# srv902/FOCUS

Hardware: AMD Instinct MI355X
Metric: clips/sec (fwd+bwd+opt step) ORViT-MF 16x224 (higher is better)
Workload: dtype bf16; 1 GPU; ORViT-Motionformer 16x224, 4 objects, batch=8 per GPU (BASELINE configs[1]); global_batch=8, frames=16, crop=224, objects=4, parallelism=dp1, optimizer=adamw+clipnorm

## Files before the change

focus_amd/csrc/gemm_tn_group.hip:

```cpp
#include "focus_common.h"
#include "gemm_internal.h"
#include <algorithm>

namespace {

typedef __attribute__((ext_vector_type(8))) __bf16 bf16x8;
typedef __attribute__((ext_vector_type(4))) short s16x4;
typedef __attribute__((ext_vector_type(4))) float f32x4;
typedef __attribute__((address_space(1))) const void gvoid_t;
typedef __attribute__((address_space(3))) void lvoid_t;
typedef __attribute__((address_space(3))) s16x4 lds_s16x4;

constexpr int BKM = 64;
constexpr int SUB = BKM * 256;
constexpr int NSTAGE = 3, NLOAD = 4;
constexpr int BI = 256, BJ = 128;

union Frag { bf16x8 v; s16x4 t[2]; uint32_t u[4]; };

__device__ __forceinline__ int swz(int row) { return ((row & 3) | ((row >> 1) & 4)) << 1; }
__device__ __forceinline__ int toff(int row, int col) {
    return row * 256 + ((((col >> 3)) ^ swz(row)) << 4) + (col & 4) * 2;
}
__device__ __forceinline__ bf16x8 col_frag16(const char* tile, int r0, int c0, int lane) {
    const int i = lane & 15;
    const int row = r0 + (i >> 2), col = c0 + 4 * (i & 3);
    Frag f;
    f.t[0] = __builtin_amdgcn_ds_read_tr16_b64_v4i16((lds_s16x4*)(tile + toff(row, col)));
    f.t[1] = __builtin_amdgcn_ds_read_tr16_b64_v4i16((lds_s16x4*)(tile + toff(row + 4, col)));
    return f.v;
}

struct Prob {
    const bf16_t* P;
    const bf16_t* Q;
    float* C;
    float* db;
    int64_t ldp, ldq;
    int32_t I, J, Mred, tiles_i, tiles_j, pad_;
};
constexpr int MAXP = 8;
struct GroupArgs { Prob p[MAXP]; int32_t nprob, nunits; };
struct UnitRec { int16_t prob, ti, tj, pad_; };

__global__ __launch_bounds__(64 * (BI * BJ / 4096 + NLOAD)) void gemm_tn_group_kernel(const GroupArgs ga, const UnitRec* __restrict__ units) {
    constexpr int NCONS = BI * BJ / 4096;
    constexpr int WJ = BJ / 64;
    constexpr int NSP = BI / 128, NSQ = BJ / 128, NSUBT = NSP + NSQ;
    constexpr int STAGE = NSUBT * SUB;
    constexpr int PIECES = NSUBT * 16 / NLOAD;
    extern __shared__ __attribute__((aligned(16))) char smem[];

    const int tid = threadIdx.x, lane = tid & 63;
    const int w = __builtin_amdgcn_readfirstlane(tid >> 6);
    const int nunits = ga.nunits;
    const int G = gridDim.x, xcd = blockIdx.x & 7, jwg = blockIdx.x >> 3;
    const int gx = (G >> 3) + (xcd < (G & 7) ? 1 : 0);
    const int q8 = nunits >> 3, r8 = nunits & 7;
    const int band0 = xcd < r8 ? xcd * (q8 + 1) : r8 * (q8 + 1) + (xcd - r8) * q8;
    const int band_n = q8 + (xcd < r8 ? 1 : 0);
    const int my_units = jwg < band_n ? (band_n - jwg + gx - 1) / gx : 0;
    if (my_units == 0) return;

    struct Unit { const bf16_t* P; const bf16_t* Q; float* C; float* db; int64_t ldp, ldq; int I, J, Mred, i0, j0, nk, valid_last, tj; };
    auto unit_of = [&](int i) __attribute__((always_inline)) {
        const UnitRec ur = units[band0 + jwg + i * gx];
        const int pi = __builtin_amdgcn_readfirstlane((int)ur.prob);
        Unit t;
        Prob p = ga.p[0];
#pragma unroll
        for (int k = 1; k < MAXP; ++k)
            if (pi == k) p = ga.p[k];
        t.P = p.P; t.Q = p.Q; t.C = p.C; t.db = p.db; t.ldp = p.ldp; t.ldq = p.ldq; t.I = p.I; t.J = p.J; t.Mred = p.Mred;
        t.i0 = __builtin_amdgcn_readfirstlane((int)ur.ti) * BI;
        t.tj = __builtin_amdgcn_readfirstlane((int)ur.tj);
        t.j0 = t.tj * BJ;
        t.nk = (p.Mred + BKM - 1) / BKM;
        t.valid_last = p.Mred - (t.nk - 1) * BKM;
        return t;
    };

    if (w >= NCONS) {
        const int L = w - NCONS;
        const int cpos = lane & 15, rin = lane >> 4;
        Unit cur = unit_of(0);
        int iu = 0, ikt = 0;
        auto issue = [&](int st) __attribute__((always_inline)) {
            char* sp = smem + st * STAGE;
            const int mb = ikt * BKM;
#pragma unroll
            for (int g = 0; g < PIECES; ++g) {
                const int sub = g >> 2, pi = g * NLOAD + L, row = (pi & 15) * 4 + rin;
                const int m = min(mb + row, cur.Mred - 1);
                const int ch = cpos ^ swz(row);
                const bf16_t* src;
                if (sub < NSP) src = cur.P + (int64_t)m * cur.ldp + min(cur.i0 + sub * 128 + ch * 8, cur.I - 8);
                else src = cur.Q + (int64_t)m * cur.ldq + min(cur.j0 + (sub - NSP) * 128 + ch * 8, cur.J - 8);
                __builtin_amdgcn_global_load_lds((gvoid_t*)src, (lvoid_t*)(sp + pi * 1024), 16, 0, 0);
            }
            if (++ikt == cur.nk) { ikt = 0; if (++iu < my_units) cur = unit_of(iu); }
        };
        int total = 0;
        for (int i = 0; i < my_units; ++i) total += unit_of(i).nk;
        issue(0);
        if (total > 1) {
            issue(1);
            asm volatile("s_waitcnt vmcnt(%0)" ::"n"(PIECES) : "memory");
        } else {
            asm volatile("s_waitcnt vmcnt(0)" ::: "memory");
        }
        __builtin_amdgcn_s_barrier();
        int st2 = 2;
        for (int t = 0; t < total; ++t) {
            if (t + 2 < total) {
                issue(st2);
                st2 = st2 == 2 ? 0 : st2 + 1;
                asm volatile("s_waitcnt vmcnt(%0)" ::"n"(PIECES) : "memory");
            } else {
                asm volatile("s_waitcnt vmcnt(0)" ::: "memory");
            }
            __builtin_amdgcn_s_barrier();
        }
        return;
    }

    const int wi = w / WJ, wj = w % WJ;
    const int fr = lane & 15, fq = lane >> 4;
    const int poff = (wi >> 1) * SUB, pcol = (wi & 1) * 64;
    const int qoff = (NSP + (wj >> 1)) * SUB, qcol = (wj & 1) * 64;
    f32x4 acc[4][4];
    constexpr int NA = 4 / WJ;
    f32x4 accb[NA];
    Frag ones;
    ones.u[0] = ones.u[1] = ones.u[2] = ones.u[3] = 0x3F803F80u;
    auto compute = [&](const char* stage, auto masked, int valid, bool cs) __attribute__((always_inline)) {
        const char* sp = stage + poff;
        const char* sq = stage + qoff;
#pragma unroll
        for (int ks = 0; ks < 2; ++ks) {
            bf16x8 fp[4], fqv[4];
#pragma unroll
            for (int a = 0; a < 4; ++a) fp[a] = col_frag16(sp, ks * 32 + 8 * fq, pcol + a * 16, lane);
#pragma unroll
            for (int b = 0; b < 4; ++b) fqv[b] = col_frag16(sq, ks * 32 + 8 * fq, qcol + b * 16, lane);
            if constexpr (decltype(masked)::value) {
                const int left = valid - (ks * 32 + 8 * fq);
#pragma unroll
                for (int a = 0; a < 4; ++a) {
                    Frag f; f.v = fp[a];
#pragma unroll
                    for (int e2 = 0; e2 < 4; ++e2) {
                        const uint32_t keep = (2 * e2 < left ? 0x0000ffffu : 0u) | (2 * e2 + 1 < left ? 0xffff0000u : 0u);
                        f.u[e2] &= keep;
                    }
                    fp[a] = f.v;
                }
            }
#pragma unroll
            for (int a = 0; a < 4; ++a)
#pragma unroll
                for (int b = 0; b < 4; ++b)
                    acc[a][b] = __builtin_amdgcn_mfma_f32_16x16x32_bf16(fqv[b], fp[a], acc[a][b], 0, 0, 0);
            if (cs) {
#pragma unroll
                for (int n = 0; n < NA; ++n) {
                    bf16x8 sel = fp[n];
#pragma unroll
                    for (int j = 1; j < WJ; ++j)
                        if (wj == j) sel = fp[j * NA + n];
                    accb[n] = __builtin_amdgcn_mfma_f32_16x16x32_bf16(ones.v, sel, accb[n], 0, 0, 0);
                }
            }
        }
    };

    __builtin_amdgcn_s_barrier();
    int st = 0;
    for (int cu = 0; cu < my_units; ++cu) {
        const Unit cur = unit_of(cu);
#pragma unroll
        for (int a = 0; a < 4; ++a)
#pragma unroll
            for (int b = 0; b < 4; ++b) acc[a][b] = (f32x4){0.f, 0.f, 0.f, 0.f};
        const bool want_b = cur.db != nullptr && cur.tj == 0;
#pragma unroll
        for (int n = 0; n < NA; ++n) accb[n] = (f32x4){0.f, 0.f, 0.f, 0.f};
        for (int kt = 0; kt + 1 < cur.nk; ++kt) {
            compute(smem + st * STAGE, std::false_type{}, BKM, want_b);
            st = st == 2 ? 0 : st + 1;
            __builtin_amdgcn_s_barrier();
        }
        compute(smem + st * STAGE, std::true_type{}, cur.valid_last, want_b);
        st = st == 2 ? 0 : st + 1;
        __builtin_amdgcn_s_barrier();
        if (want_b && fq == 0) {
#pragma unroll
            for (int n = 0; n < NA; ++n) {
                const int gi = cur.i0 + wi * 64 + (wj * NA + n) * 16 + fr;
                if (gi < cur.I) cur.db[gi] = accb[n][0];
            }
        }
#pragma unroll
        for (int a = 0; a < 4; ++a) {
            const int gi = cur.i0 + wi * 64 + a * 16 + fr;
            if (gi >= cur.I) continue;
#pragma unroll
            for (int b = 0; b < 4; ++b) {
                const int gj = cur.j0 + wj * 64 + b * 16 + fq * 4;
                if (gj < cur.J)
                    *reinterpret_cast<float4*>(cur.C + (int64_t)gi * cur.J + gj) =
                        make_float4(acc[a][b][0], acc[a][b][1], acc[a][b][2], acc[a][b][3]);
            }
        }
    }
}

}

extern "C" int focus_linear_wgrad_group_units(const focus_wgrad_item* items, int n_items) {
    if (!items || n_items <= 0) return 0;
    int64_t t = 0;
    for (int p = 0; p < n_items; ++p) t += (int64_t)((items[p].N + BI - 1) / BI) * ((items[p].K + BJ - 1) / BJ);
    return t > 0x7fffffff ? -1 : (int)t;
}

extern "C" int focus_linear_wgrad_group_plan(const focus_wgrad_item* items, int n_items, void* host_units, size_t bytes) {
    if (!items || !host_units) return FOCUS_ERR_NULL;
    if (n_items <= 0 || n_items > MAXP) return FOCUS_ERR_SHAPE;
    const int total = focus_linear_wgrad_group_units(items, n_items);
    if (total <= 0 || bytes < (size_t)total * sizeof(UnitRec)) return FOCUS_ERR_WORKSPACE;
    UnitRec* u = static_cast<UnitRec*>(host_units);
    constexpr int BA = 4, BB = 8;
    int n = 0;
    for (int p = 0; p < n_items; ++p) {
        const int ti_n = (items[p].N + BI - 1) / BI, tj_n = (items[p].K + BJ - 1) / BJ;
        for (int bi = 0; bi < ti_n; bi += BA)
            for (int bj = 0; bj < tj_n; bj += BB)
                for (int ti = bi; ti < std::min(bi + BA, ti_n); ++ti)
                    for (int tj = bj; tj < std::min(bj + BB, tj_n); ++tj)
                        u[n++] = UnitRec{(int16_t)p, (int16_t)ti, (int16_t)tj, 0};
    }
    return n == total ? FOCUS_OK : FOCUS_ERR_SHAPE;
}

extern "C" int focus_linear_wgrad_group(const focus_wgrad_item* items, int n_items, const void* dev_units, void* stream) {
    if (!items || !dev_units) return FOCUS_ERR_NULL;
    if (n_items <= 0) return FOCUS_OK;
    if (n_items > MAXP) return FOCUS_ERR_SHAPE;
    GroupArgs ga = {};
    int units = 0;
    for (int p = 0; p < n_items; ++p) {
        const focus_wgrad_item& it = items[p];
        if (!it.dy || !it.x || !it.dw) return FOCUS_ERR_NULL;
        if (it.M <= 0 || it.N < 8 || it.K < 8 || (it.N & 7) || (it.K & 7) || (it.ld_dy & 7) || (it.ld_x & 7)) return FOCUS_ERR_SHAPE;
        if (!focus_aligned(it.dy, 16) || !focus_aligned(it.x, 16) || !focus_aligned(it.dw, 16)) return FOCUS_ERR_ALIGN;
        Prob& q = ga.p[p];
        q.P = static_cast<const bf16_t*>(it.dy); q.Q = static_cast<const bf16_t*>(it.x);
        q.C = it.dw; q.db = it.db; q.ldp = it.ld_dy; q.ldq = it.ld_x;
        q.I = it.N; q.J = it.K; q.Mred = it.M;
        q.tiles_i = (it.N + BI - 1) / BI; q.tiles_j = (it.K + BJ - 1) / BJ; q.pad_ = 0;
        if (q.tiles_i > 32767 || q.tiles_j > 32767) return FOCUS_ERR_SHAPE;
        units += q.tiles_i * q.tiles_j;
    }
    ga.nprob = n_items;
    ga.nunits = units;
    hipStream_t s = static_cast<hipStream_t>(stream);
    const size_t lds = (size_t)NSTAGE * (BI / 128 + BJ / 128) * SUB;
    auto k = gemm_tn_group_kernel;
    static bool once = (hipFuncSetAttribute((const void*)k, hipFuncAttributeMaxDynamicSharedMemorySize, lds) == hipSuccess);
    (void)once;
    hipLaunchKernelGGL(k, dim3(std::min(units, 256)), dim3(64 * (BI * BJ / 4096 + NLOAD)), lds, s, ga,
                       static_cast<const UnitRec*>(dev_units));
    FOCUS_CHECK_LAUNCH();
    return FOCUS_OK;
}
```

Baseline: 299.1 clips/s.

## Precompute loader offsets, index problem table via kernarg, stage epilogue through LDS

The loader waves now compute per-row byte offsets once per unit and advance them by a fixed stride each k-step, clamping rows only on the last tile. This removes the per-load index arithmetic and the upfront pass that summed all units' k-tiles. The problem table is read directly from the kernel-argument segment using scalar reads instead of a select chain, and the bias path is made a compile-time branch. The output epilogue goes through a per-wave swizzled LDS slab so stores become coalesced nontemporal row writes, at the cost of extra LDS and waits.

Result: faster. 306.5 clips/s (median of 6 runs) (+2.5%).

```diff
diff --git a/focus_amd/csrc/gemm_tn_group.hip b/focus_amd/csrc/gemm_tn_group.hip
--- a/focus_amd/csrc/gemm_tn_group.hip
+++ b/focus_amd/csrc/gemm_tn_group.hip
@@ -1,6 +1,7 @@
 #include "focus_common.h"
 #include "gemm_internal.h"
 #include <algorithm>
+#include <cstddef>
 
 namespace {
 
@@ -15,6 +16,7 @@
 constexpr int SUB = BKM * 256;
 constexpr int NSTAGE = 3, NLOAD = 4;
 constexpr int BI = 256, BJ = 128;
+constexpr int SLAB = 2048;
 
 union Frag { bf16x8 v; s16x4 t[2]; uint32_t u[4]; };
 
@@ -29,6 +31,11 @@
     f.t[0] = __builtin_amdgcn_ds_read_tr16_b64_v4i16((lds_s16x4*)(tile + toff(row, col)));
     f.t[1] = __builtin_amdgcn_ds_read_tr16_b64_v4i16((lds_s16x4*)(tile + toff(row + 4, col)));
     return f.v;
+}
+
+__device__ __forceinline__ uint64_t uni64(uint64_t v) {
+    return ((uint64_t)(uint32_t)__builtin_amdgcn_readfirstlane((int)(v >> 32)) << 32) |
+           (uint32_t)__builtin_amdgcn_readfirstlane((int)(uint32_t)v);
 }
 
 struct Prob {
@@ -64,62 +71,116 @@
 
     struct Unit { const bf16_t* P; const bf16_t* Q; float* C; float* db; int64_t ldp, ldq; int I, J, Mred, i0, j0, nk, valid_last, tj; };
     auto unit_of = [&](int i) __attribute__((always_inline)) {
-        const UnitRec ur = units[band0 + jwg + i * gx];
-        const int pi = __builtin_amdgcn_readfirstlane((int)ur.prob);
+        const uint2 raw = reinterpret_cast<const uint2*>(units)[band0 + jwg + i * gx];
+        const int pi = __builtin_amdgcn_readfirstlane((int)(raw.x & 0xffffu)) & (MAXP - 1);
         Unit t;
-        Prob p = ga.p[0];
-#pragma unroll
-        for (int k = 1; k < MAXP; ++k)
-            if (pi == k) p = ga.p[k];
-        t.P = p.P; t.Q = p.Q; t.C = p.C; t.db = p.db; t.ldp = p.ldp; t.ldq = p.ldq; t.I = p.I; t.J = p.J; t.Mred = p.Mred;
-        t.i0 = __builtin_amdgcn_readfirstlane((int)ur.ti) * BI;
-        t.tj = __builtin_amdgcn_readfirstlane((int)ur.tj);
+        static_assert(offsetof(GroupArgs, p) == 0, "the problem table must open the kernel-argument segment");
+        typedef __attribute__((address_space(4))) const Prob karg_prob_t;
+        const karg_prob_t& p = ((const karg_prob_t*)__builtin_amdgcn_kernarg_segment_ptr())[pi];
+        t.P = reinterpret_cast<const bf16_t*>(uni64(reinterpret_cast<uint64_t>(p.P)));
+        t.Q = reinterpret_cast<const bf16_t*>(uni64(reinterpret_cast<uint64_t>(p.Q)));
+        t.C = reinterpret_cast<float*>(uni64(reinterpret_cast<uint64_t>(p.C)));
+        t.db = reinterpret_cast<float*>(uni64(reinterpret_cast<uint64_t>(p.db)));
+        t.ldp = (int64_t)uni64((uint64_t)p.ldp); t.ldq = (int64_t)uni64((uint64_t)p.ldq);
+        t.I = __builtin_amdgcn_readfirstlane(p.I); t.J = __builtin_amdgcn_readfirstlane(p.J);
+        t.Mred = __builtin_amdgcn_readfirstlane(p.Mred);
+        t.i0 = __builtin_amdgcn_readfirstlane((int)(raw.x >> 16)) * BI;
+        t.tj = __builtin_amdgcn_readfirstlane((int)(raw.y & 0xffffu));
         t.j0 = t.tj * BJ;
-        t.nk = (p.Mred + BKM - 1) / BKM;
-        t.valid_last = p.Mred - (t.nk - 1) * BKM;
+        t.nk = (t.Mred + BKM - 1) / BKM;
+        t.valid_last = t.Mred - (t.nk - 1) * BKM;
         return t;
     };
 
     if (w >= NCONS) {
         const int L = w - NCONS;
         const int cpos = lane & 15, rin = lane >> 4;
-        Unit cur = unit_of(0);
+        constexpr int GP = NSP * 4, GQ = NSQ * 4;
+        uint32_t p_off[GP], q_off[GQ];
+        const char* p_cur = nullptr;
+        const char* q_cur = nullptr;
+        int64_t p_step = 0, q_step = 0;
+        uint32_t ldp2 = 0, ldq2 = 0;
+        int nk = 0, Mred = 0;
         int iu = 0, ikt = 0;
+        bool more = true;
+        auto rowk = [&](int k) __attribute__((always_inline)) { return (k * NLOAD + L) * 4 + rin; };
+        auto setup = [&](int i) __attribute__((always_inline)) {
+            const Unit t = unit_of(i);
+            p_cur = reinterpret_cast<const char*>(t.P);
+            q_cur = reinterpret_cast<const char*>(t.Q);
+            p_step = t.ldp * (2 * BKM);
+            q_step = t.ldq * (2 * BKM);
+            ldp2 = 2u * (uint32_t)t.ldp;
+            ldq2 = 2u * (uint32_t)t.ldq;
+            nk = t.nk;
+            Mred = t.Mred;
+#pragma unroll
+            for (int k = 0; k < 4; ++k) {
+                const int row = rowk(k), ch = cpos ^ swz(row);
+#pragma unroll
+                for (int s = 0; s < NSP; ++s)
+                    p_off[s * 4 + k] = (uint32_t)row * ldp2 + 2u * (uint32_t)min(t.i0 + s * 128 + ch * 8, t.I - 8);
+#pragma unroll
+                for (int s = 0; s < NSQ; ++s)
+                    q_off[s * 4 + k] = (uint32_t)row * ldq2 + 2u * (uint32_t)min(t.j0 + s * 128 + ch * 8, t.J - 8);
+            }
+        };
         auto issue = [&](int st) __attribute__((always_inline)) {
             char* sp = smem + st * STAGE;
-            const int mb = ikt * BKM;
-#pragma unroll
-            for (int g = 0; g < PIECES; ++g) {
-                const int sub = g >> 2, pi = g * NLOAD + L, row = (pi & 15) * 4 + rin;
-                const int m = min(mb + row, cur.Mred - 1);
-                const int ch = cpos ^ swz(row);
-                const bf16_t* src;
-                if (sub < NSP) src = cur.P + (int64_t)m * cur.ldp + min(cur.i0 + sub * 128 + ch * 8, cur.I - 8);
-                else src = cur.Q + (int64_t)m * cur.ldq + min(cur.j0 + (sub - NSP) * 128 + ch * 8, cur.J - 8);
-                __builtin_amdgcn_global_load_lds((gvoid_t*)src, (lvoid_t*)(sp + pi * 1024), 16, 0, 0);
-            }
-            if (++ikt == cur.nk) { ikt = 0; if (++iu < my_units) cur = unit_of(iu); }
+            if (ikt + 1 < nk) {
+#pragma unroll
+                for (int g = 0; g < GP; ++g)
+                    __builtin_amdgcn_global_load_lds((gvoid_t*)(p_cur + p_off[g]), (lvoid_t*)(sp + (g * NLOAD + L) * 1024), 16, 0, 0);
+#pragma unroll
+                for (int g = 0; g < GQ; ++g)
+                    __builtin_amdgcn_global_load_lds((gvoid_t*)(q_cur + q_off[g]), (lvoid_t*)(sp + ((GP + g) * NLOAD + L) * 1024), 16, 0, 0);
+                p_cur += p_step;
+                q_cur += q_step;
+                ++ikt;
+            } else {
+                const int last = Mred - 1 - ikt * BKM;
+                uint32_t pb[4], qb[4];
+#pragma unroll
+                for (int k = 0; k < 4; ++k) {
+                    const uint32_t over = (uint32_t)max(rowk(k) - last, 0);
+                    pb[k] = over * ldp2;
+                    qb[k] = over * ldq2;
+                }
+#pragma unroll
+                for (int g = 0; g < GP; ++g)
+                    __builtin_amdgcn_global_load_lds((gvoid_t*)(p_cur + (p_off[g] - pb[g & 3])), (lvoid_t*)(sp + (g * NLOAD + L) * 1024), 16, 0, 0);
+#pragma unroll
+                for (int g = 0; g < GQ; ++g)
+                    __builtin_amdgcn_global_load_lds((gvoid_t*)(q_cur + (q_off[g] - qb[g & 3])), (lvoid_t*)(sp + ((GP + g) * NLOAD + L) * 1024), 16, 0, 0);
+                ikt = 0;
+                if (++iu < my_units) setup(iu);
+                else more = false;
+            }
         };
-        int total = 0;
-        for (int i = 0; i < my_units; ++i) total += unit_of(i).nk;
+        setup(0);
         issue(0);
-        if (total > 1) {
+        int pending = 1;
+        if (more) {
             issue(1);
+            ++pending;
             asm volatile("s_waitcnt vmcnt(%0)" ::"n"(PIECES) : "memory");
         } else {
             asm volatile("s_waitcnt vmcnt(0)" ::: "memory");
         }
         __builtin_amdgcn_s_barrier();
         int st2 = 2;
-        for (int t = 0; t < total; ++t) {
-            if (t + 2 < total) {
+        while (pending > 0) {
+            if (more) {
                 issue(st2);
+                ++pending;
                 st2 = st2 == 2 ? 0 : st2 + 1;
                 asm volatile("s_waitcnt vmcnt(%0)" ::"n"(PIECES) : "memory");
             } else {
                 asm volatile("s_waitcnt vmcnt(0)" ::: "memory");
             }
             __builtin_amdgcn_s_barrier();
+            --pending;
         }
         return;
     }
@@ -133,7 +194,7 @@
     f32x4 accb[NA];
     Frag ones;
     ones.u[0] = ones.u[1] = ones.u[2] = ones.u[3] = 0x3F803F80u;
-    auto compute = [&](const char* stage, auto masked, int valid, bool cs) __attribute__((always_inline)) {
+    auto compute = [&](const char* stage, auto masked, int valid, auto cs) __attribute__((always_inline)) {
         const char* sp = stage + poff;
         const char* sq = stage + qoff;
 #pragma unroll
@@ -161,7 +222,7 @@
 #pragma unroll
                 for (int b = 0; b < 4; ++b)
                     acc[a][b] = __builtin_amdgcn_mfma_f32_16x16x32_bf16(fqv[b], fp[a], acc[a][b], 0, 0, 0);
-            if (cs) {
+            if constexpr (decltype(cs)::value) {
 #pragma unroll
                 for (int n = 0; n < NA; ++n) {
                     bf16x8 sel = fp[n];
@@ -185,14 +246,18 @@
         const bool want_b = cur.db != nullptr && cur.tj == 0;
 #pragma unroll
         for (int n = 0; n < NA; ++n) accb[n] = (f32x4){0.f, 0.f, 0.f, 0.f};
-        for (int kt = 0; kt + 1 < cur.nk; ++kt) {
-            compute(smem + st * STAGE, std::false_type{}, BKM, want_b);
+        auto stream = [&](auto wb) __attribute__((always_inline)) {
+            for (int kt = 0; kt + 1 < cur.nk; ++kt) {
+                compute(smem + st * STAGE, std::false_type{}, BKM, wb);
+                st = st == 2 ? 0 : st + 1;
+                __builtin_amdgcn_s_barrier();
+            }
+            compute(smem + st * STAGE, std::true_type{}, cur.valid_last, wb);
             st = st == 2 ? 0 : st + 1;
             __builtin_amdgcn_s_barrier();
-        }
-        compute(smem + st * STAGE, std::true_type{}, cur.valid_last, want_b);
-        st = st == 2 ? 0 : st + 1;
-        __builtin_amdgcn_s_barrier();
+        };
+        if (want_b) stream(std::true_type{});
+        else stream(std::false_type{});
         if (want_b && fq == 0) {
 #pragma unroll
             for (int n = 0; n < NA; ++n) {
@@ -200,16 +265,24 @@
                 if (gi < cur.I) cur.db[gi] = accb[n][0];
             }
         }
+        char* slab = smem + NSTAGE * STAGE + w * SLAB;
+        const int srow = lane >> 3, sch = lane & 7;
 #pragma unroll
         for (int a = 0; a < 4; ++a) {
-            const int gi = cur.i0 + wi * 64 + a * 16 + fr;
-            if (gi >= cur.I) continue;
-#pragma unroll
-            for (int b = 0; b < 4; ++b) {
-                const int gj = cur.j0 + wj * 64 + b * 16 + fq * 4;
-                if (gj < cur.J)
-                    *reinterpret_cast<float4*>(cur.C + (int64_t)gi * cur.J + gj) =
-                        make_float4(acc[a][b][0], acc[a][b][1], acc[a][b][2], acc[a][b][3]);
+#pragma unroll
+            for (int h = 0; h < 2; ++h) {
+#pragma unroll
+                for (int bb = 0; bb < 2; ++bb)
+                    *reinterpret_cast<f32x4*>(slab + fr * 128 + (((bb * 4 + fq) ^ ((fr >> 1) & 7)) << 4)) = acc[a][h * 2 + bb];
+                asm volatile("s_waitcnt lgkmcnt(0)" ::: "memory");
+#pragma unroll
+                for (int p8 = 0; p8 < 2; ++p8) {
+                    const int row = p8 * 8 + srow;
+                    const f32x4 v = *reinterpret_cast<const f32x4*>(slab + row * 128 + ((sch ^ ((row >> 1) & 7)) << 4));
+                    const int gi = cur.i0 + wi * 64 + a * 16 + row, gj = cur.j0 + wj * 64 + h * 32 + sch * 4;
+                    if (gi < cur.I && gj < cur.J) __builtin_nontemporal_store(v, reinterpret_cast<f32x4*>(cur.C + (int64_t)gi * cur.J + gj));
+                }
+                asm volatile("s_waitcnt lgkmcnt(0)" ::: "memory");
             }
         }
     }
@@ -246,6 +319,7 @@
 extern "C" int focus_linear_wgrad_group(const focus_wgrad_item* items, int n_items, const void* dev_units, void* stream) {
     if (!items || !dev_units) return FOCUS_ERR_NULL;
     if (n_items <= 0) return FOCUS_OK;
+    if (!focus_aligned(dev_units, 8)) return FOCUS_ERR_ALIGN;
     if (n_items > MAXP) return FOCUS_ERR_SHAPE;
     GroupArgs ga = {};
     int units = 0;
@@ -254,6 +328,7 @@
         if (!it.dy || !it.x || !it.dw) return FOCUS_ERR_NULL;
         if (it.M <= 0 || it.N < 8 || it.K < 8 || (it.N & 7) || (it.K & 7) || (it.ld_dy & 7) || (it.ld_x & 7)) return FOCUS_ERR_SHAPE;
         if (!focus_aligned(it.dy, 16) || !focus_aligned(it.x, 16) || !focus_aligned(it.dw, 16)) return FOCUS_ERR_ALIGN;
+        if (it.ld_dy <= 0 || it.ld_x <= 0 || it.ld_dy > (1 << 24) || it.ld_x > (1 << 24)) return FOCUS_ERR_SHAPE;
         Prob& q = ga.p[p];
         q.P = static_cast<const bf16_t*>(it.dy); q.Q = static_cast<const bf16_t*>(it.x);
         q.C = it.dw; q.db = it.db; q.ldp = it.ld_dy; q.ldq = it.ld_x;
@@ -265,7 +340,7 @@
     ga.nprob = n_items;
     ga.nunits = units;
     hipStream_t s = static_cast<hipStream_t>(stream);
-    const size_t lds = (size_t)NSTAGE * (BI / 128 + BJ / 128) * SUB;
+    const size_t lds = (size_t)NSTAGE * (BI / 128 + BJ / 128) * SUB + (size_t)(BI * BJ / 4096) * SLAB;
     auto k = gemm_tn_group_kernel;
     static bool once = (hipFuncSetAttribute((const void*)k, hipFuncAttributeMaxDynamicSharedMemorySize, lds) == hipSuccess);
     (void)once;
```
